# thucz/splatter360

Measured on AMD Instinct MI355X. Metric: Msplats/s fwd+bwd @1M Gaussians, 1024x512 ERP, higher is better.
Workload: dtype f32; 1 GPU; BASELINE configs[2]: 1048576 encoder-like synthetic Gaussians (seed 0, deg-4 SH, from 2 context panoramas 1024x512), 1024x512 ERP = 6 faces 256x256 + stitch, fwdbwd, L2 loss on faces (fused epilogue, scalar reduced in the backward's first launch), lean tile lists; gaussians=1048576, face=256, views_per_gpu=1, parallelism=view-sharded x1, num_rendered=2237238, visible_pairs=1096454, split_lists=auto, split_quadrants=0, wide_rectangles=0, workspace_bytes_forward=1086434304, workspace_bytes_backward=1062934272, max_instances=2862083

## Files before the change

### splatter360_amd/csrc/s360_device.h

```cpp
#pragma once
#include <hip/hip_runtime.h>
#include <stdint.h>

#include "../../include/s360.h"

#define S360_WAVE 64
#define S360_BLOCK 256

#ifndef S360_SUB_W
#define S360_SUB_W 8
#endif

static inline int s360_effective_degree(const S360Params* prm) {
    return (prm->sh_degree > 3 && (prm->flags & S360_FLAG_SH_DEG4_IGNORED)) ? 3 : prm->sh_degree;
}

#ifndef S360_PREC_F4
#define S360_PREC_F4 4
#endif

namespace s360 {

constexpr int PREC_F4 = S360_PREC_F4;
constexpr int SUB_W = S360_SUB_W, SUB_H = 64 / S360_SUB_W;
// ... 11 lines not shown
#define S360_SEG_LEN 512
#endif
#ifndef S360_SEG_HEAD
#define S360_SEG_HEAD 1024
#endif
#ifndef S360_SEG_BWD_BLOCKS
#define S360_SEG_BWD_BLOCKS 256
#endif
#ifndef S360_SEG_MIN_REST
#define S360_SEG_MIN_REST 512
#endif
constexpr uint32_t SEG_LEN = S360_SEG_LEN, SEG_HEAD = S360_SEG_HEAD, SEG_MIN_REST = S360_SEG_MIN_REST, SEG_PER_CHUNK = 4096 / SEG_LEN;
constexpr uint32_t SEG_K0 = SEG_HEAD / SEG_LEN;
static_assert(4096 % SEG_LEN == 0 && SEG_HEAD % SEG_LEN == 0 && SEG_LEN % 64 == 0 && SEG_K0 >= 1, "segments tile the sort's 4 096-key chunks; slot 0 holds the head's state");
__device__ constexpr float SEG_T_FAR = 1.0f / 16.0f;
__host__ __device__ inline size_t seg_slots(size_t cap) { return (size_t)SEG_PER_CHUNK * (cap / 2048 + 1); }
__host__ __device__ inline size_t seg_slots_of(const S360Params* prm) {
    return prm->max_segments ? (size_t)prm->max_segments : seg_slots(prm->max_instances ? prm->max_instances : 1);
}
#define S360_HDR_SPLIT 5
#define S360_HDR_SEGWORK 6
#define S360_HDR_TILES_DONE 24
#define S360_HDR_NLONG 25
#define S360_SEG_CLAIM 0x80000000u
#define S360_HDR_SEGBUFS 32

inline int device_cu_count() {
    static int cached[64] = {};
    int dev = 0;
    if (hipGetDevice(&dev) != hipSuccess || dev < 0 || dev >= 64) return 256;
    if (!cached[dev]) {
        int n = 0;
        if (hipDeviceGetAttribute(&n, hipDeviceAttributeMultiprocessorCount, dev) != hipSuccess || n <= 0) { (void)hipGetLastError(); n = 256; }
        cached[dev] = n;
    }
    return cached[dev];
}

inline int resident_blocks(const void* fn, int block_threads, int slot) {
    static int cached[64][16] = {};
    int dev = 0;
    if (hipGetDevice(&dev) != hipSuccess || dev < 0 || dev >= 64 || slot < 0 || slot >= 16) return 4 * 256;
    if (!cached[dev][slot]) {
        int per_cu = 0;
        if (hipOccupancyMaxActiveBlocksPerMultiprocessor(&per_cu, fn, block_threads, 0) != hipSuccess || per_cu <= 0) { (void)hipGetLastError(); per_cu = 4; }
        cached[dev][slot] = per_cu * device_cu_count();
// ... 573 lines not shown
```

### splatter360_amd/csrc/s360_forward.hip

```cpp
#include "s360_device.h"
#include "s360_prof.h"
#include "s360_adapter_math.h"

#include <cstdio>
#include <cstdlib>

namespace s360 {

typedef float f4v __attribute__((ext_vector_type(4)));

template <bool CH_MAJOR, bool JAC>
__global__ __launch_bounds__(S360_BLOCK) void k_sh_eval(KParams kp, const S360View* __restrict__ views,
                                                       const float* __restrict__ means, const float* __restrict__ shs,
                                                       float4* __restrict__ rgbc, float* __restrict__ sh_jac,
                                                       uint32_t* __restrict__ zero_ptr, int zero_words) {
    const int g = blockIdx.x * S360_BLOCK + threadIdx.x;
    if (g < zero_words) zero_ptr[g] = 0u;
    if (g >= kp.P) return;
    const bool fast = kp.M == 25 && kp.deg == 4;
    const float* sh = shs + (size_t)g * kp.M * 3;
    float c[75];
    if (fast) load75(sh, c);
    const S360View& vw = views[0];
    const float sc = vw.scale;
// ... 610 lines not shown
    if (lane == 63) lds[wave] = inc;
    __syncthreads();
    uint32_t base = 0, tot = 0;
#pragma unroll
    for (int w = 0; w < NW; ++w) {
        const uint32_t s = lds[w];
        if (w < wave) base += s;
        tot += s;
    }
    __syncthreads();
    total = tot;
    return base + inc - v;
}

#ifndef S360_SORT_THREADS
#define S360_SORT_THREADS 512
#endif
constexpr int SORT_THREADS = S360_SORT_THREADS;
constexpr uint32_t SORT_SHORT = 2048;
constexpr uint32_t SORT_CHUNK = 8 * SORT_THREADS;
static_assert(SORT_SHORT % SORT_THREADS == 0 && SORT_SHORT <= SORT_CHUNK, "short lists: SORT_SHORT / SORT_THREADS keys per thread");
constexpr uint32_t MAX_PASSES = 4;
__device__ __forceinline__ uint32_t ceil_log2_u32(uint32_t x) { return x <= 1 ? 0u : 32u - (uint32_t)__builtin_clz(x - 1); }
constexpr uint32_t LDSM_CHUNKS = 4;
constexpr int LDSM_E = 32;
__device__ __forceinline__ uint32_t merge_passes_of(uint32_t nch) { return nch <= 1 ? 0u : nch <= LDSM_CHUNKS ? 1u : ceil_log2_u32(nch); }

struct SegBufs {
    const uint32_t* chunk_start;
    uint32_t* seg_flag;
    uint32_t* seg_arrive;
    uint32_t* seg_arrive2;
    uint32_t n_slots;
    float4* part_c;
    float* part_t;
    float* part_e;
    uint32_t* part_l;
    uint32_t* part_n;
    float4* seg_c;
    float* seg_t;
    uint32_t* seg_cnt;
    uint2* seg_info;
    uint32_t* header;
};
static_assert(sizeof(SegBufs) <= (64 - S360_HDR_SEGBUFS) * 4, "SegBufs is parked in the workspace header");

constexpr int TS_BLOCK = 1024;
__global__ __launch_bounds__(TS_BLOCK) void k_tile_scan(const uint32_t* __restrict__ tile_count, uint32_t* __restrict__ tile_start,
                                                         uint32_t* __restrict__ tile_cursor, uint32_t* __restrict__ tile_max_contrib,
// ... 35 lines not shown
            tile_max_contrib[i1] = 0;
            chunk_start[i1] = ccarry + cex1;
        }
        carry += tot;
        ccarry += ctot;
    }
    atomicMax(&lds_max, mx);
    __syncthreads();
    if (threadIdx.x == 0) {
        chunk_start[nt] = ccarry;
        tile_start[nt] = carry;
        header[0] = carry;
        header[1] = carry > cap ? 1u : 0u;
        header[2] = lds_max;
        {
            const uint32_t nmax = min(lds_max, cap);
            const uint32_t nch = nmax > SORT_SHORT ? (nmax + SORT_CHUNK - 1) / SORT_CHUNK : 0u;
            header[3] = merge_passes_of(nch);
        }
        header[4] = 0;
        *reinterpret_cast<SegBufs*>(header + S360_HDR_SEGBUFS) = sg_in;
        header[S360_HDR_SPLIT] = 0;
        header[6] = header[7] = 0;
        if (header_mirror) __hip_atomic_store(header_mirror, (unsigned long long)carry | ((unsigned long long)(carry > cap ? 1u : 0u) << 32) |
                                                             ((unsigned long long)ccarry << 33),
                                              __ATOMIC_RELAXED, __HIP_MEMORY_SCOPE_SYSTEM);
        header[S360_HDR_NLONG] = lds_nlong;
        for (int i = 8; i < 25; ++i) header[i] = 0;
    }
}

#ifndef S360_EMIT_PPT
#define S360_EMIT_PPT 4
#endif
constexpr int EMIT_PPT = S360_EMIT_PPT;

template <bool LDS_BIN, bool COOP = false>
__global__ __launch_bounds__(S360_BLOCK) void k_emit(KParams kp, const uint32_t* __restrict__ tiles_touched,
                                                    const uint8_t* __restrict__ vis_mask, const float4* __restrict__ recA, const float4* __restrict__ recC,
                                                    const float* __restrict__ depths, const uint32_t* __restrict__ tile_start,
                                                    uint32_t* __restrict__ tile_cursor, uint64_t* __restrict__ keys,
                                                    uint2* __restrict__ slot_info, uint32_t* __restrict__ slot_pair,
                                                    uint32_t* __restrict__ slot_ticket, uint32_t* __restrict__ header,
                                                    uint32_t* __restrict__ long_pairs) {
    extern __shared__ __attribute__((aligned(16))) uint32_t lds_bin[];
    __shared__ uint32_t s_scan[S360_BLOCK / 64];
// ... 130 lines not shown
                    m = (m >> 1) | 0x80000000u;
                }
        }
        if (COOP) {
            for (unsigned long long big = __ballot(wide); big; big &= big - 1ull) {
                const int src = (int)__builtin_ctzll(big);
                const uint32_t lo = (uint32_t)__shfl((int)rlo[j], src), hi = (uint32_t)__shfl((int)rhi[j], src);
                const uint32_t ps = (uint32_t)__shfl((int)p, src), ds = (uint32_t)__shfl((int)dbits[j], src), s0 = (uint32_t)__shfl((int)slot, src);
                const uint64_t key = ((uint64_t)ds << 32) | (uint64_t)ps;
                const int minx = lo & 0xFFFFu, miny = lo >> 16, w = (int)(hi & 0xFFFFu) - minx, n = w * ((int)(hi >> 16) - miny);
                for (int i = lane; i < n; i += 64) {
                    const int y = i / w;
                    const int t = (miny + y) * kp.gx + minx + (i - y * w);
                    const uint32_t pos = LDS_BIN ? base[t] + atomicAdd(&cnt[t], 1u)
                                                 : tile_start[tb + t] + atomicAdd(&tile_cursor[tb + t], 1u);
                    if (pos < kp.cap) keys[pos] = key;
                    if (slot_pair && s0 + (uint32_t)i < kp.cap) slot_pair[s0 + (uint32_t)i] = ps | 0x80000000u;
                }
            }
        }
    }
}

template <int THREADS, int E>
__device__ __forceinline__ void block_merge_sort(const uint64_t* __restrict__ in, uint64_t* __restrict__ out,
                                                 uint32_t* __restrict__ list, uint32_t n, uint64_t* lds_m) {
#define S360_PHYS(i) ((i) + (i) / E)
    const int tid = threadIdx.x;
    uint64_t k[E];
#pragma unroll
    for (int q = 0; q < E; ++q) {
        const uint32_t i = (uint32_t)(tid * E + q);
        k[q] = i < n ? in[i] : ~0ull;
    }
#pragma unroll
    for (int r = 0; r < E; ++r) {
#pragma unroll
        for (int q = (r & 1); q + 1 < E; q += 2) {
            const uint64_t a = k[q], b = k[q + 1];
            k[q] = a < b ? a : b;
            k[q + 1] = a < b ? b : a;
        }
    }
#pragma unroll
    for (int q = 0; q < E; ++q) lds_m[S360_PHYS((uint32_t)(tid * E + q))] = k[q];
#define S360_SORT_SYNC(w)                                                      \
    do {                                                                       \
// ... 33 lines not shown
                    ka = a < width ? S360_A(a) : ~0ull;
                } else {
                    ++b;
                    kb = b < width ? S360_B(b) : ~0ull;
                }
            }
        }
        S360_SORT_SYNC(width);
        if (live) {
#pragma unroll
            for (int q = 0; q < E; ++q) lds_m[S360_PHYS(out0 + q)] = k[q];
        }
        S360_SORT_SYNC(2u * width);
#undef S360_A
#undef S360_B
    }
    __syncthreads();
#undef S360_SORT_SYNC
#pragma unroll
    for (int q = 0; q < E; ++q) {
        const uint32_t i = (uint32_t)(tid * E + q);
        if (i < n) {
            const uint64_t kq = lds_m[S360_PHYS(i)];
            out[i] = kq;
            if (list) list[i] = (uint32_t)kq;
        }
    }
#undef S360_PHYS
}



struct ChunkUnit {
    uint32_t s, n, k, passes, t;
    bool valid;
};
__device__ __forceinline__ ChunkUnit chunk_unit(const uint32_t* __restrict__ tile_start, const uint32_t* __restrict__ chunk_start,
                                                 int nt, uint32_t cap, uint32_t b) {
    ChunkUnit u;
    u.valid = b < chunk_start[nt];
    u.s = u.n = u.k = u.passes = u.t = 0;
    if (!u.valid) return u;
    const int lane = threadIdx.x & 63;
    int lo = 0, hi = nt;
    while (hi - lo > 1) {
        const int step = (hi - lo + 63) / 64;
        const int t = lo + lane * step;
        const bool p = t < hi && chunk_start[t] <= b;
        const int cnt = __popcll(__ballot(p));
        const int nhi = lo + cnt * step;
        lo = lo + (cnt - 1) * step;
        hi = nhi < hi ? nhi : hi;
    }
    u.s = min(tile_start[lo], cap);
    u.n = min(tile_start[lo + 1], cap) - u.s;
    u.k = b - chunk_start[lo];
    u.t = (uint32_t)lo;
    u.passes = merge_passes_of((u.n + SORT_CHUNK - 1) / SORT_CHUNK);
    return u;
}

__global__ __launch_bounds__(SORT_THREADS) void k_sort_stage1(const uint32_t* __restrict__ tile_start, const uint32_t* __restrict__ chunk_start,
                                                    int nt, uint64_t* __restrict__ keys, uint64_t* __restrict__ alt,
                                                    uint32_t* __restrict__ list, uint32_t cap, uint32_t max_passes, uint32_t cgrid,
                                                    const uint32_t* __restrict__ tile_count, uint32_t* __restrict__ tile_order,
                                                    const uint32_t* __restrict__ header, unsigned long long* __restrict__ wide_mirror) {
    extern __shared__ __attribute__((aligned(16))) uint64_t lds_m[];
    const uint32_t bid = blockIdx.x;
    if (bid < cgrid) {
        const uint32_t nchunks = chunk_start[nt];
        for (uint32_t b = bid; b < nchunks; b += cgrid) {
            const ChunkUnit u = chunk_unit(tile_start, chunk_start, nt, cap, b);
            if (u.valid && u.passes <= max_passes) {
                const uint32_t c0 = u.k * SORT_CHUNK, len = min(SORT_CHUNK, u.n - c0);
                uint64_t* dst = ((u.passes & 1u) ? alt : keys) + u.s + c0;
                block_merge_sort<SORT_THREADS, 8>(keys + u.s + c0, dst, u.passes == 0 ? list + u.s : nullptr, len, lds_m);
            }
            __syncthreads();
        }
        return;
    }
    if (bid < cgrid + (uint32_t)nt) {
        const uint32_t tile = bid - cgrid;
        const uint32_t s = min(tile_start[tile], cap), e = min(tile_start[tile + 1], cap);
        const uint32_t n = e - s;
        if (n == 0 || n > SORT_SHORT) return;
        block_merge_sort<SORT_THREADS, (int)(SORT_SHORT / SORT_THREADS)>(keys + s, keys + s, list + s, n, lds_m);
        return;
    }
    if (wide_mirror && threadIdx.x == 0) __hip_atomic_store(wide_mirror, (unsigned long long)header[4], __ATOMIC_RELAXED, __HIP_MEMORY_SCOPE_SYSTEM);
    if (tile_order) order_units_body<SORT_THREADS>(tile_count, tile_order, nt);
}

__device__ __forceinline__ uint64_t ld_dev(const uint64_t* p) { return __hip_atomic_load(p, __ATOMIC_RELAXED, __HIP_MEMORY_SCOPE_AGENT); }
__device__ __forceinline__ void st_dev(uint64_t* p, uint64_t v) { __hip_atomic_store(p, v, __ATOMIC_RELAXED, __HIP_MEMORY_SCOPE_AGENT); }

__device__ __forceinline__ uint32_t merge_path_global_wave(const uint64_t* __restrict__ A, uint32_t la,
                                                           const uint64_t* __restrict__ B, uint32_t lb, uint32_t d, int lane) {
    uint32_t lo = d > lb ? d - lb : 0u, hi = d < la ? d : la;
    while (lo < hi) {
        const uint32_t step = (hi - lo + 63u) / 64u;
        const uint32_t a = lo + (uint32_t)lane * step;
        const bool p = a < hi && ld_dev(A + a) <= ld_dev(B + (d - 1 - a));
        const uint32_t cnt = (uint32_t)__popcll(__ballot(p));
        if (cnt == 0) {
            hi = lo;
        } else {
            const uint32_t nhi = lo + cnt * step;
            lo = lo + (cnt - 1) * step + 1;
            hi = nhi < hi ? nhi : hi;
        }
    }
    return lo;
}

#ifndef S360_MERGE_GRID
#define S360_MERGE_GRID 256
#endif
__device__ __forceinline__ void merge_unit(const ChunkUnit& u, uint32_t pass, const uint64_t* __restrict__ keys_c, uint64_t* __restrict__ keys,
                                           uint64_t* __restrict__ alt, uint32_t* __restrict__ list, uint64_t* lds_m, uint32_t* s_part) {
    constexpr int THREADS = SORT_THREADS, E = 8;
#define S360_PHYS(i) ((i) + (i) / E)
    (void)keys_c;
    const uint32_t R = SORT_CHUNK << pass;
    const uint32_t o_tile = u.k * SORT_CHUNK, len = min(SORT_CHUNK, u.n - o_tile);
    const uint32_t pair0 = o_tile / (2 * R) * (2 * R);
    const uint32_t la = min(R, u.n - pair0), lb = min(R, u.n - pair0 - la);
    const uint64_t* src = (((u.passes - pass) & 1u) ? alt : keys) + u.s + pair0;
    uint64_t* dst = (((u.passes - pass - 1) & 1u) ? alt : keys) + u.s + o_tile;
    const uint64_t* A = src;
    const uint64_t* B = src + la;
    const uint32_t o = o_tile - pair0;
    if (threadIdx.x < 128) {
        const int w = threadIdx.x >> 6;
        const uint32_t r = merge_path_global_wave(A, la, B, lb, o + (uint32_t)w * len, threadIdx.x & 63);
        if ((threadIdx.x & 63) == 0) s_part[w] = r;
    }
    __syncthreads();
    const uint32_t a0 = s_part[0], a1 = s_part[1], b0 = o - a0, b1 = o + len - a1;
    const uint32_t na = a1 - a0, nb = b1 - b0;
    {
        uint64_t kin[E];
#pragma unroll
        for (int q = 0; q < E; ++q) {
            const uint32_t i = (uint32_t)threadIdx.x + (uint32_t)q * THREADS;
            kin[q] = i < len ? ld_dev(i < na ? A + (a0 + i) : B + (b0 + (i - na))) : 0ull;
// ... 16 lines not shown
        uint64_t ka = a < na ? lds_m[S360_PHYS(a)] : ~0ull, kb = b < nb ? lds_m[S360_PHYS(na + b)] : ~0ull;
        const bool last_pass = pass + 1 == u.passes;
        uint32_t* lst = list + u.s + o_tile;
#pragma unroll
        for (int q = 0; q < E; ++q) {
            const bool take_a = ka <= kb;
            const uint64_t kq = take_a ? ka : kb;
            if (take_a) {
                ++a;
                ka = a < na ? lds_m[S360_PHYS(a)] : ~0ull;
            } else {
                ++b;
                kb = b < nb ? lds_m[S360_PHYS(na + b)] : ~0ull;
            }
            if (out0 + q < len) {
                st_dev(dst + (out0 + q), kq);
                if (last_pass) lst[out0 + q] = (uint32_t)kq;
            }
        }
    }
#undef S360_PHYS
}

static_assert(SORT_THREADS * LDSM_E == (int)(LDSM_CHUNKS * SORT_CHUNK), "a thread merges LDSM_E outputs per pass");
constexpr size_t LDSM_LDS_BYTES = (size_t)(LDSM_CHUNKS * SORT_CHUNK + LDSM_CHUNKS * SORT_CHUNK / LDSM_E) * 8;
__device__ __forceinline__ void merge_tile_lds(uint32_t n, const uint64_t* __restrict__ src, uint64_t* __restrict__ dst, uint32_t* __restrict__ lst,
                                               uint64_t* lds_m) {
    constexpr int E = LDSM_E;
#define S360_PHYS(i) ((i) + (i) / E)
    {
        uint64_t k[E];
#pragma unroll
        for (int q = 0; q < E; ++q) {
            const uint32_t i = (uint32_t)threadIdx.x + (uint32_t)q * SORT_THREADS;
            k[q] = i < n ? src[i] : 0ull;
        }
#pragma unroll
        for (int q = 0; q < E; ++q) {
            const uint32_t i = (uint32_t)threadIdx.x + (uint32_t)q * SORT_THREADS;
            if (i < n) lds_m[S360_PHYS(i)] = k[q];
        }
    }
    __syncthreads();
    const uint32_t out0 = (uint32_t)threadIdx.x * E;
    for (uint32_t width = SORT_CHUNK; width < n; width <<= 1) {
        uint64_t k[E];
        if (out0 < n) {
            const uint32_t pa = out0 / (2 * width) * (2 * width), pb = pa + width;
            const uint32_t la = min(width, n - pa), lb = pb < n ? min(width, n - pb) : 0u;
            const uint32_t diag = out0 - pa;
            uint32_t lo = diag > lb ? diag - lb : 0u, hi = diag < la ? diag : la;
            while (lo < hi) {
                const uint32_t mid = (lo + hi) >> 1;
                if (lds_m[S360_PHYS(pa + mid)] <= lds_m[S360_PHYS(pb + (diag - 1 - mid))]) lo = mid + 1; else hi = mid;
            }
            uint32_t a = lo, b = diag - lo;
            uint64_t ka = a < la ? lds_m[S360_PHYS(pa + a)] : ~0ull, kb = b < lb ? lds_m[S360_PHYS(pb + b)] : ~0ull;
#pragma unroll
            for (int q = 0; q < E; ++q) {
                const bool take_a = ka <= kb;
                k[q] = take_a ? ka : kb;
                if (take_a) {
                    ++a;
                    ka = a < la ? lds_m[S360_PHYS(pa + a)] : ~0ull;
                } else {
                    ++b;
                    kb = b < lb ? lds_m[S360_PHYS(pb + b)] : ~0ull;
                }
            }
        }
        __syncthreads();
        if (out0 < n) {
#pragma unroll
            for (int q = 0; q < E; ++q)
                if (out0 + q < n) lds_m[S360_PHYS(out0 + q)] = k[q];
        }
        __syncthreads();
    }
    {
        uint64_t k[E];
#pragma unroll
        for (int q = 0; q < E; ++q) {
            const uint32_t i = (uint32_t)threadIdx.x + (uint32_t)q * SORT_THREADS;
            k[q] = i < n ? lds_m[S360_PHYS(i)] : 0ull;
        }
#pragma unroll
        for (int q = 0; q < E; ++q) {
            const uint32_t i = (uint32_t)threadIdx.x + (uint32_t)q * SORT_THREADS;
            if (i < n) {
                dst[i] = k[q];
                lst[i] = (uint32_t)k[q];
            }
        }
    }
#undef S360_PHYS
}

template <int THREADS>
__device__ __forceinline__ void sort_tiles_global_body(const uint32_t* __restrict__ tile_start, uint64_t* __restrict__ keys,
                                                       uint32_t* __restrict__ list, uint32_t lo, uint32_t cap, int nt) {
  for (int tile = blockIdx.x; tile < nt; tile += gridDim.x) {
    const uint32_t s = min(tile_start[tile], cap), e = min(tile_start[tile + 1], cap);
    const uint32_t n = e - s;
    if (n <= lo) continue;
    uint32_t npad = 1;
    while (npad < n) npad <<= 1;
    uint64_t* kk = keys + s;
    for (uint32_t k = 2; k <= npad; k <<= 1) {
        const uint32_t half = k >> 1;
        for (uint32_t t = threadIdx.x; t < (npad >> 1); t += THREADS) {
            const uint32_t blk = t / half, off = t - blk * half;
            const uint32_t i = blk * k + off, l = blk * k + (k - 1 - off);
            if (l < n) {
                const uint64_t a = kk[i], b = kk[l];
                if (a > b) {
                    kk[i] = b;
                    kk[l] = a;
                }
            }
        }
        __threadfence_block();
        __syncthreads();
        for (uint32_t j = k >> 2; j > 0; j >>= 1) {
            for (uint32_t t = threadIdx.x; t < (npad >> 1); t += THREADS) {
                const uint32_t i = ((t & ~(j - 1)) << 1) | (t & (j - 1)), l = i | j;
                if (l < n) {
                    const uint64_t a = kk[i], b = kk[l];
                    if (a > b) {
                        kk[i] = b;
                        kk[l] = a;
                    }
                }
            }
            __threadfence_block();
            __syncthreads();
        }
    }
    for (uint32_t i = threadIdx.x; i < n; i += THREADS) list[s + i] = (uint32_t)kk[i];
    __syncthreads();
  }
}

__global__ __launch_bounds__(SORT_THREADS) void k_merge_all(const uint32_t* __restrict__ tile_start, const uint32_t* __restrict__ chunk_start,
                                                  int nt, uint64_t* __restrict__ keys, uint64_t* __restrict__ alt,
                                                  uint32_t* __restrict__ list, uint32_t cap, uint32_t max_passes,
                                                  const uint32_t* __restrict__ header, uint32_t* __restrict__ merge_done,
                                                  uint32_t global_lo) {
    extern __shared__ __attribute__((aligned(16))) uint64_t lds_m[];
    __shared__ uint32_t s_part[2];
    __shared__ uint32_t s_ticket;
    const uint32_t npass = min(header[3], max_passes);
    const uint32_t nchunks = npass ? chunk_start[nt] : 0u;
    const uint32_t nunits = npass * nchunks;
    uint32_t* const queue = merge_done + (size_t)nt * MAX_PASSES;
    for (;;) {
        if (threadIdx.x == 0) s_ticket = nunits ? __hip_atomic_fetch_add(queue, 1u, __ATOMIC_RELAXED, __HIP_MEMORY_SCOPE_AGENT) : 0u;
        __syncthreads();
        const uint32_t tk = s_ticket;
        __syncthreads();
        if (tk >= nunits) break;
        const uint32_t pass = tk / nchunks, blk = tk - pass * nchunks;
        const ChunkUnit u = chunk_unit(tile_start, chunk_start, nt, cap, blk);
        if (!u.valid || u.passes > max_passes || pass >= u.passes) continue;
        const uint32_t nch = (u.n + SORT_CHUNK - 1) / SORT_CHUNK;
        if (nch <= LDSM_CHUNKS) {
            if (u.k == 0) merge_tile_lds(u.n, alt + u.s, keys + u.s, list + u.s, lds_m);
            continue;
        }
        if (pass > 0) {
            if (threadIdx.x == 0) {
                while (__hip_atomic_load(&merge_done[(size_t)u.t * MAX_PASSES + pass - 1], __ATOMIC_RELAXED, __HIP_MEMORY_SCOPE_AGENT) < nch)
                    __builtin_amdgcn_s_sleep(4);
            }
            __syncthreads();
        }
        merge_unit(u, pass, keys, keys, alt, list, lds_m, s_part);
        asm volatile("s_waitcnt vmcnt(0)" ::: "memory");
        __builtin_amdgcn_fence(__ATOMIC_RELEASE, "workgroup");
        __syncthreads();
        if (threadIdx.x == 0 && pass + 1 < u.passes)
            __hip_atomic_fetch_add(&merge_done[(size_t)u.t * MAX_PASSES + pass], 1u, __ATOMIC_RELAXED, __HIP_MEMORY_SCOPE_AGENT);
    }
    if (header[2] > global_lo) sort_tiles_global_body<SORT_THREADS>(tile_start, keys, list, global_lo, cap, nt);
}

#ifndef S360_SPARSE_PIXELS
#define S360_SPARSE_PIXELS 6
#endif
constexpr int SPARSE_PIXELS = S360_SPARSE_PIXELS;

struct MseEp {
    const float* target;
    float* d_images;
    float* partials;
    float grad_scale;
    float* loss_out;
};

__global__ __launch_bounds__(MSE_BLOCK) void k_mse_finish(const float* __restrict__ partials, int n_per_view, int V, float loss_scale,
                                                         float inv_elems, float* __restrict__ out) {
    mse_finish_body(partials, n_per_view, V, loss_scale, inv_elems, out);
}


__device__ __forceinline__ void st_dev32(uint32_t* p, uint32_t v) { __hip_atomic_store(p, v, __ATOMIC_RELAXED, __HIP_MEMORY_SCOPE_AGENT); }
__device__ __forceinline__ uint32_t ld_dev32(const uint32_t* p) { return __hip_atomic_load(p, __ATOMIC_RELAXED, __HIP_MEMORY_SCOPE_AGENT); }
// ... 183 lines not shown
    }
}

template <bool WITH_DEPTH, bool COH>
__device__ __forceinline__ void seg_item(const KParams& kp, const S360View* __restrict__ views, const uint32_t* __restrict__ tile_start,
                                         const uint32_t* __restrict__ list, const float4* __restrict__ recA, float* __restrict__ images,
                                         float* __restrict__ final_T, uint32_t* __restrict__ n_contrib, uint32_t* __restrict__ tile_max_contrib,
                                         uint32_t* __restrict__ strip_last, const float* __restrict__ depths, float* __restrict__ depth_maps,
                                         int depth_mode, const MseEp& ep, float4* __restrict__ surv, uint32_t* __restrict__ surv_count,
                                         const SegBufs& sg, int nt, uint32_t* __restrict__ dbg, const WaveLds& L, int lane, uint2 item, uint32_t wi,
                                         uint32_t nwork);

#ifndef S360_SPLIT_WAVES
#define S360_SPLIT_WAVES 4
#endif
#ifndef S360_P1_GRID
#define S360_P1_GRID 1024
#endif
#ifndef S360_P1_FIRST
#define S360_P1_FIRST 0
#endif
#ifndef S360_P2_GRID
#define S360_P2_GRID 1024
#endif
#ifndef S360_SEGS_SPINS
#define S360_SEGS_SPINS 600
#endif
template <bool WITH_DEPTH, bool SPLIT>
__global__ __launch_bounds__(S360_BLOCK) __attribute__((amdgpu_waves_per_eu(SPLIT ? S360_SPLIT_WAVES : 6, SPLIT ? S360_SPLIT_WAVES : 6))) void k_render(KParams kp, const S360View* __restrict__ views,
                                                      const uint32_t* __restrict__ tile_start, const uint32_t* __restrict__ list,
                                                      const float4* __restrict__ recA, const float4* __restrict__ recB,
                                                      const float4* __restrict__ recC, float* __restrict__ images,
                                                      float* __restrict__ final_T, uint32_t* __restrict__ n_contrib,
                                                      uint32_t* __restrict__ tile_max_contrib, uint32_t* __restrict__ strip_last,
                                                      uint32_t* __restrict__ dbg, const float* __restrict__ depths,
                                                      float* __restrict__ depth_maps, int depth_mode, MseEp ep,
                                                      const uint32_t* __restrict__ tile_order, float4* __restrict__ surv,
                                                      uint32_t* __restrict__ surv_count, uint32_t* __restrict__ hdr_loss,
                                                      const SegBufs* __restrict__ sgp, const uint32_t* __restrict__ chunk_start,
                                                      unsigned long long* __restrict__ cand_mirror, int nt, const uint32_t* __restrict__ list_all,
                                                      const float* __restrict__ depths_all) {
#ifdef S360_DBG_TIMING
    const long long t_begin = wall_clock64();
#endif
    __shared__ __attribute__((aligned(16))) float s_x[S360_BLOCK / 64][68], s_y[S360_BLOCK / 64][68], s_a[S360_BLOCK / 64][68],
        s_b[S360_BLOCK / 64][68], s_c[S360_BLOCK / 64][68], s_o[S360_BLOCK / 64][68];
    __shared__ __attribute__((aligned(16))) float2 s_rg[S360_BLOCK / 64][68], s_bz[S360_BLOCK / 64][68];
    __shared__ __attribute__((aligned(16))) uint32_t s_pos[S360_BLOCK / 64][68];
    if (hdr_loss && blockIdx.x == 0 && threadIdx.x == 0) {
// ... 651 lines not shown
    const size_t np = (size_t)prm->V * (size_t)(prm->P > 0 ? prm->P : 1);
    const size_t gx = (prm->W + 15) / 16, gy = (prm->H + 15) / 16;
    const size_t nt = (size_t)prm->V * gx * gy;
    const size_t cap = prm->max_instances ? prm->max_instances : 1;
    const size_t npix = (size_t)prm->V * prm->H * prm->W;
    const bool fwd_only = (prm->flags & S360_FLAG_FORWARD_ONLY) != 0;
    size_t o = 0;
    auto take = [&](size_t bytes) {
        size_t r = o;
        o = align_up(o + bytes);
        return r;
    };
    out->header = take(64 * 4);
    out->tiles_touched = take(np * 4);
    out->vis_mask = take((size_t)(prm->P > 0 ? prm->P : 1));
    out->slot_base = take(np * 8);
    out->rec_a = take(np * 48);
    out->rec_b = out->rec_a + 16;
    out->rec_c = out->rec_a + 32;
    out->clamped = take(np);
    out->depths = take(np * 4);
    out->tile_count = take(nt * 4);
    out->slot_ticket = take((size_t)prm->V * 256);
    out->merge_done = take((nt * MAX_PASSES + 1) * 4);
    out->seg_flag = take(nt * 4 * 4);
    out->seg_arrive = take(nt * 4 * 4);
    out->seg_arrive2 = take((nt * 4 + 1) * 4);
    out->tile_start = take((nt + 1) * 4);
    out->tile_cursor = take(nt * 4);
    out->chunk_start = take((nt + 1) * 4);
    out->tile_order = take(nt * 4);
    out->keys = take(cap * 8);
    out->keys_alt = take(cap * 8);
    out->list = take(cap * 4);
    out->final_T = take(npix * 4);
    out->n_contrib = take(npix * 4);
    out->tile_max_contrib = take(nt * 4);
    out->strip_last = take(nt * 4 * 4);
    out->slot_pair = take(cap * 4);
    out->long_pairs = take(fwd_only ? 16 : (cap / 32 + 1) * 4);
    out->rgbc = take((size_t)(prm->P > 0 ? prm->P : 1) * 16);
    out->sh_jac = take((size_t)(prm->P > 0 ? prm->P : 1) * 36);
    out->surv = take(fwd_only ? 16 : cap * 4 * 48);
    out->surv_count = take(nt * 4 * 4);
    {
        const bool split = (prm->flags & S360_FLAG_SPLIT_LISTS) != 0;
        const size_t ns = split ? seg_slots_of(prm) : 1, nl = ns * 4 * 64;
// ... 159 lines not shown
    if (kp.P > 0) {
        const dim3 egrid((kp.P + S360_BLOCK * EMIT_PPT - 1) / (S360_BLOCK * EMIT_PPT), kp.V);
        uint32_t* slot_pair = (kp.flags & S360_FLAG_FORWARD_ONLY) ? nullptr : (uint32_t*)(ws + L.slot_pair);
        {
        ProfScope ps(PS_EMIT, st);
        if ((size_t)kp.T * 8 <= 64 * 1024 && (kp.flags & S360_FLAG_COOP_WALK))
            hipLaunchKernelGGL((k_emit<true, true>), egrid, dim3(S360_BLOCK), (size_t)kp.T * 8, st, kp, tiles_touched, vis_mask, recA, recC,
                               depths, tile_start, tile_cursor, keys, slot_info, slot_pair, slot_ticket, header, (uint32_t*)(ws + L.long_pairs));
        else if ((size_t)kp.T * 8 <= 64 * 1024)
            hipLaunchKernelGGL(k_emit<true>, egrid, dim3(S360_BLOCK), (size_t)kp.T * 8, st, kp, tiles_touched, vis_mask, recA, recC,
                               depths, tile_start, tile_cursor, keys, slot_info, slot_pair, slot_ticket, header, (uint32_t*)(ws + L.long_pairs));
        else
            hipLaunchKernelGGL(k_emit<false>, egrid, dim3(S360_BLOCK), 0, st, kp, tiles_touched, vis_mask, recA, recC, depths, tile_start,
                               tile_cursor, keys, slot_info, slot_pair, slot_ticket, header, (uint32_t*)(ws + L.long_pairs));
        }
        S360_CHECK_LAUNCH();
        ProfScope ps(PS_SORT, st);
        {
            const size_t cap_keys = kp.cap < (uint32_t)kp.P ? kp.cap : (size_t)kp.P;
            uint32_t passes = 0;
            while (passes < MAX_PASSES && ((size_t)SORT_CHUNK << passes) < cap_keys) ++passes;
            const uint32_t global_lo = SORT_CHUNK << passes;
            const unsigned cgrid = (unsigned)min((size_t)1024, (size_t)kp.cap / SORT_CHUNK + (size_t)kp.cap / SORT_SHORT + 2);
            const size_t lds512 = (size_t)(SORT_CHUNK + SORT_CHUNK / 8) * 8;
            hipLaunchKernelGGL(k_sort_stage1, dim3(cgrid + nt + 1), dim3(SORT_THREADS), lds512, st, tile_start, chunk_start, nt, keys, keys_alt, list,
                               kp.cap, passes, cgrid, tile_count, tile_order, header,
                               prm->header_mirror ? (unsigned long long*)prm->header_mirror + 2 : (unsigned long long*)nullptr);
            if (passes > 0) {
                const unsigned mgrid = cgrid < (unsigned)S360_MERGE_GRID ? cgrid : (unsigned)S360_MERGE_GRID;
                {
                    static bool attr_done[64] = {};
                    int dev = 0;
                    if (hipGetDevice(&dev) == hipSuccess && dev >= 0 && dev < 64 && !attr_done[dev]) {
                        (void)hipFuncSetAttribute((const void*)k_merge_all, hipFuncAttributeMaxDynamicSharedMemorySize, (int)LDSM_LDS_BYTES);
                        (void)hipGetLastError();
                        attr_done[dev] = true;
                    }
                }
                hipLaunchKernelGGL(k_merge_all, dim3(mgrid), dim3(SORT_THREADS), LDSM_LDS_BYTES, st, tile_start, chunk_start, nt, keys, keys_alt, list,
                                   kp.cap, passes, header, (uint32_t*)(ws + L.merge_done), (size_t)global_lo < cap_keys ? global_lo : 0xFFFFFFFFu);
            }
        }
        S360_CHECK_LAUNCH();
    }
    {
        ProfScope ps(PS_RENDER, st);
        const dim3 rgrid(nt), rblock(S360_BLOCK);
        const bool training = !(kp.flags & S360_FLAG_FORWARD_ONLY);
        float4* surv = training ? (float4*)(ws + L.surv) : nullptr;
        uint32_t* surv_count = training ? (uint32_t*)(ws + L.surv_count) : nullptr;
#ifdef S360_DBG_TIMING
        uint32_t* dbg = (uint32_t*)keys_alt;
#else
        uint32_t* dbg = header + 8;
#endif
        const bool defer = training && kp.P > 0 && ep.target && ep.loss_out && (kp.flags & S360_FLAG_DEFER_LOSS);
        uint32_t* hdr_loss = defer ? header + S360_HDR_LOSS : nullptr;
        const bool split = kp.P > 0 && (kp.flags & S360_FLAG_SPLIT_LISTS);
        SegBufs sg{split ? chunk_start : (const uint32_t*)nullptr, (uint32_t*)(ws + L.seg_flag), (uint32_t*)(ws + L.seg_arrive),
                   (uint32_t*)(ws + L.seg_arrive2), (uint32_t)seg_slots_of(prm),
                   (float4*)(ws + L.part_c), (float*)(ws + L.part_t), (float*)(ws + L.part_e), (uint32_t*)(ws + L.part_l), (uint32_t*)(ws + L.part_n),
                   (float4*)(ws + L.seg_c), (float*)(ws + L.seg_t), (uint32_t*)(ws + L.seg_cnt), (uint2*)(ws + L.seg_info), header};
        unsigned long long* cand = prm->header_mirror ? (unsigned long long*)prm->header_mirror + 1 : nullptr;
        const SegBufs* sgp = split ? (const SegBufs*)(header + S360_HDR_SEGBUFS) : (const SegBufs*)nullptr;
// ... 75 lines not shown
```

### splatter360_amd/rasterizer.py

```python
from __future__ import annotations

import ctypes as C
import os
from typing import NamedTuple, Optional

import torch
from torch import Tensor, nn

from . import _lib

VIEW_FLOATS = 44

SH_DEG4_IGNORED = bool(int(os.environ.get("S360_SH_DEG4_IGNORED", "0")))


class GaussianRasterizationSettings(NamedTuple):
    image_height: int
    image_width: int
    tanfovx: float
    tanfovy: float
    bg: Tensor
    scale_modifier: float
    viewmatrix: Tensor
    projmatrix: Tensor
# ... 237 lines not shown

    def count_contributions(self):
        out = torch.zeros(2, dtype=torch.int64, device=self.workspace.device)
        with torch.cuda.device(self.workspace.device):
            stream = C.c_void_p(torch.cuda.current_stream(self.workspace.device).cuda_stream)
            _lib.check(_lib.lib().s360_count_contributions(C.byref(self.prm), _ptr(self.workspace), self.layout.total_bytes, _ptr(out), stream),
                       "s360_count_contributions")
        a, b = out.cpu().tolist()
        return int(a), int(b)

    def count_backward_slots(self) -> dict:
        out = torch.zeros(32, dtype=torch.int64, device=self.workspace.device)
        with torch.cuda.device(self.workspace.device):
            stream = C.c_void_p(torch.cuda.current_stream(self.workspace.device).cuda_stream)
            _lib.check(_lib.lib().s360_count_backward_slots(C.byref(self.prm), _ptr(self.workspace), self.layout.total_bytes, _ptr(out), stream),
                       "s360_count_backward_slots")
        c = [int(x) for x in out.cpu().tolist()]
        return dict(executed=c[0], padding=c[1], stopped=c[2], miss=c[3], contributing=c[4], skipped_runs=c[5], units=c[6], groups=c[7],
                    by_unit_hit_decile=c[8:18], runs_by_active_records=dict(zip(("0", "1-4", "5-8", "9-16", "17-24", "25-32", "33-48", "49-64"), c[18:26])),
                    records=c[29], reach_upper_half=c[26], reach_lower_half=c[27], reach_both_halves=c[28], half_wave_iterations=c[30])

    def split_errors(self) -> int:
        return int(self.header()[7].item())

    def mopup_items(self) -> int:
        n = int(self.header()[6].item())
        if n == 0:
            return 0
        second = self._arr(self.layout.seg_info, 2 * n, torch.int32).view(n, 2)[:, 1].to(torch.int64)
        return int(((second & 0x80000000) == 0).sum().item())

    def num_rendered(self) -> int:
        return self._read_header()[0]

    def overflowed(self) -> bool:
        return self._read_header()[1]


def _ptr(t: Optional[Tensor]):
    return None if t is None else C.c_void_p(t.data_ptr())


def _f32c(t: Tensor, name: str) -> Tensor:
    if not t.is_cuda:
        raise RuntimeError(f"{name} must live on the GPU (hip device); the rasteriser has no CPU path")
    return t.detach().float().contiguous()
# ... 502 lines not shown
```

Baseline: 1359 Msplats/s.

## Fuse chunk sort and merge passes into one persistent kernel with per-tile readiness counters

Folds the separate merge kernel into the stage-1 sort launch. Dedicated merge blocks now spin on per-tile counters of sorted chunks, so merging of a long tile can begin as soon as its chunks are sorted rather than after a kernel boundary. The LDS-resident small-merge path (merge_tile_lds) is removed, and every multi-chunk tile now goes through the global merge-path passes. Spin timeouts record an error in the header, which adds a risk of aborted merges or of deadlock if merge blocks are resident while chunk blocks are not yet scheduled.

Result: faster. 1380 Msplats/s, median of 6 (+1.5%).

```diff
diff --git a/splatter360_amd/csrc/s360_device.h b/splatter360_amd/csrc/s360_device.h
--- a/splatter360_amd/csrc/s360_device.h
+++ b/splatter360_amd/csrc/s360_device.h
@@ -57,6 +57,8 @@
 #define S360_HDR_SEGWORK 6
 #define S360_HDR_TILES_DONE 24
 #define S360_HDR_NLONG 25
+#define S360_HDR_SORT_ERR_TILE 26
+#define S360_HDR_SORT_ERR_PASS 27
 #define S360_SEG_CLAIM 0x80000000u
 #define S360_HDR_SEGBUFS 32
 
diff --git a/splatter360_amd/csrc/s360_forward.hip b/splatter360_amd/csrc/s360_forward.hip
--- a/splatter360_amd/csrc/s360_forward.hip
+++ b/splatter360_amd/csrc/s360_forward.hip
@@ -656,9 +656,10 @@
 static_assert(SORT_SHORT % SORT_THREADS == 0 && SORT_SHORT <= SORT_CHUNK, "short lists: SORT_SHORT / SORT_THREADS keys per thread");
 constexpr uint32_t MAX_PASSES = 4;
 __device__ __forceinline__ uint32_t ceil_log2_u32(uint32_t x) { return x <= 1 ? 0u : 32u - (uint32_t)__builtin_clz(x - 1); }
-constexpr uint32_t LDSM_CHUNKS = 4;
-constexpr int LDSM_E = 32;
-__device__ __forceinline__ uint32_t merge_passes_of(uint32_t nch) { return nch <= 1 ? 0u : nch <= LDSM_CHUNKS ? 1u : ceil_log2_u32(nch); }
+__device__ __forceinline__ uint32_t merge_passes_of(uint32_t nch) { return ceil_log2_u32(nch); }
+#ifndef S360_SEGS_SPINS
+#define S360_SEGS_SPINS 600
+#endif
 
 struct SegBufs {
     const uint32_t* chunk_start;
@@ -740,6 +741,7 @@
         *reinterpret_cast<SegBufs*>(header + S360_HDR_SEGBUFS) = sg_in;
         header[S360_HDR_SPLIT] = 0;
         header[6] = header[7] = 0;
+        header[S360_HDR_SORT_ERR_TILE] = header[S360_HDR_SORT_ERR_PASS] = 0;
         if (header_mirror) __hip_atomic_store(header_mirror, (unsigned long long)carry | ((unsigned long long)(carry > cap ? 1u : 0u) << 32) |
                                                              ((unsigned long long)ccarry << 33),
                                               __ATOMIC_RELAXED, __HIP_MEMORY_SCOPE_SYSTEM);
@@ -916,7 +918,10 @@
     }
 }
 
-template <int THREADS, int E>
+__device__ __forceinline__ uint64_t ld_dev(const uint64_t* p) { return __hip_atomic_load(p, __ATOMIC_RELAXED, __HIP_MEMORY_SCOPE_AGENT); }
+__device__ __forceinline__ void st_dev(uint64_t* p, uint64_t v) { __hip_atomic_store(p, v, __ATOMIC_RELAXED, __HIP_MEMORY_SCOPE_AGENT); }
+
+template <int THREADS, int E, bool DEV = false>
 __device__ __forceinline__ void block_merge_sort(const uint64_t* __restrict__ in, uint64_t* __restrict__ out,
                                                  uint32_t* __restrict__ list, uint32_t n, uint64_t* lds_m) {
 #define S360_PHYS(i) ((i) + (i) / E)
@@ -996,13 +1001,12 @@
         const uint32_t i = (uint32_t)(tid * E + q);
         if (i < n) {
             const uint64_t kq = lds_m[S360_PHYS(i)];
-            out[i] = kq;
+            if (DEV) st_dev(out + i, kq); else out[i] = kq;
             if (list) list[i] = (uint32_t)kq;
         }
     }
 #undef S360_PHYS
 }
-
 
 
 struct ChunkUnit {
@@ -1034,41 +1038,6 @@
     return u;
 }
 
-__global__ __launch_bounds__(SORT_THREADS) void k_sort_stage1(const uint32_t* __restrict__ tile_start, const uint32_t* __restrict__ chunk_start,
-                                                    int nt, uint64_t* __restrict__ keys, uint64_t* __restrict__ alt,
-                                                    uint32_t* __restrict__ list, uint32_t cap, uint32_t max_passes, uint32_t cgrid,
-                                                    const uint32_t* __restrict__ tile_count, uint32_t* __restrict__ tile_order,
-                                                    const uint32_t* __restrict__ header, unsigned long long* __restrict__ wide_mirror) {
-    extern __shared__ __attribute__((aligned(16))) uint64_t lds_m[];
-    const uint32_t bid = blockIdx.x;
-    if (bid < cgrid) {
-        const uint32_t nchunks = chunk_start[nt];
-        for (uint32_t b = bid; b < nchunks; b += cgrid) {
-            const ChunkUnit u = chunk_unit(tile_start, chunk_start, nt, cap, b);
-            if (u.valid && u.passes <= max_passes) {
-                const uint32_t c0 = u.k * SORT_CHUNK, len = min(SORT_CHUNK, u.n - c0);
-                uint64_t* dst = ((u.passes & 1u) ? alt : keys) + u.s + c0;
-                block_merge_sort<SORT_THREADS, 8>(keys + u.s + c0, dst, u.passes == 0 ? list + u.s : nullptr, len, lds_m);
-            }
-            __syncthreads();
-        }
-        return;
-    }
-    if (bid < cgrid + (uint32_t)nt) {
-        const uint32_t tile = bid - cgrid;
-        const uint32_t s = min(tile_start[tile], cap), e = min(tile_start[tile + 1], cap);
-        const uint32_t n = e - s;
-        if (n == 0 || n > SORT_SHORT) return;
-        block_merge_sort<SORT_THREADS, (int)(SORT_SHORT / SORT_THREADS)>(keys + s, keys + s, list + s, n, lds_m);
-        return;
-    }
-    if (wide_mirror && threadIdx.x == 0) __hip_atomic_store(wide_mirror, (unsigned long long)header[4], __ATOMIC_RELAXED, __HIP_MEMORY_SCOPE_SYSTEM);
-    if (tile_order) order_units_body<SORT_THREADS>(tile_count, tile_order, nt);
-}
-
-__device__ __forceinline__ uint64_t ld_dev(const uint64_t* p) { return __hip_atomic_load(p, __ATOMIC_RELAXED, __HIP_MEMORY_SCOPE_AGENT); }
-__device__ __forceinline__ void st_dev(uint64_t* p, uint64_t v) { __hip_atomic_store(p, v, __ATOMIC_RELAXED, __HIP_MEMORY_SCOPE_AGENT); }
-
 __device__ __forceinline__ uint32_t merge_path_global_wave(const uint64_t* __restrict__ A, uint32_t la,
                                                            const uint64_t* __restrict__ B, uint32_t lb, uint32_t d, int lane) {
     uint32_t lo = d > lb ? d - lb : 0u, hi = d < la ? d : la;
@@ -1088,14 +1057,10 @@
     return lo;
 }
 
-#ifndef S360_MERGE_GRID
-#define S360_MERGE_GRID 256
-#endif
-__device__ __forceinline__ void merge_unit(const ChunkUnit& u, uint32_t pass, const uint64_t* __restrict__ keys_c, uint64_t* __restrict__ keys,
+__device__ __forceinline__ void merge_unit(const ChunkUnit& u, uint32_t pass, uint64_t* __restrict__ keys,
                                            uint64_t* __restrict__ alt, uint32_t* __restrict__ list, uint64_t* lds_m, uint32_t* s_part) {
     constexpr int THREADS = SORT_THREADS, E = 8;
 #define S360_PHYS(i) ((i) + (i) / E)
-    (void)keys_c;
     const uint32_t R = SORT_CHUNK << pass;
     const uint32_t o_tile = u.k * SORT_CHUNK, len = min(SORT_CHUNK, u.n - o_tile);
     const uint32_t pair0 = o_tile / (2 * R) * (2 * R);
@@ -1158,84 +1123,11 @@
 #undef S360_PHYS
 }
 
-static_assert(SORT_THREADS * LDSM_E == (int)(LDSM_CHUNKS * SORT_CHUNK), "a thread merges LDSM_E outputs per pass");
-constexpr size_t LDSM_LDS_BYTES = (size_t)(LDSM_CHUNKS * SORT_CHUNK + LDSM_CHUNKS * SORT_CHUNK / LDSM_E) * 8;
-__device__ __forceinline__ void merge_tile_lds(uint32_t n, const uint64_t* __restrict__ src, uint64_t* __restrict__ dst, uint32_t* __restrict__ lst,
-                                               uint64_t* lds_m) {
-    constexpr int E = LDSM_E;
-#define S360_PHYS(i) ((i) + (i) / E)
-    {
-        uint64_t k[E];
-#pragma unroll
-        for (int q = 0; q < E; ++q) {
-            const uint32_t i = (uint32_t)threadIdx.x + (uint32_t)q * SORT_THREADS;
-            k[q] = i < n ? src[i] : 0ull;
-        }
-#pragma unroll
-        for (int q = 0; q < E; ++q) {
-            const uint32_t i = (uint32_t)threadIdx.x + (uint32_t)q * SORT_THREADS;
-            if (i < n) lds_m[S360_PHYS(i)] = k[q];
-        }
-    }
-    __syncthreads();
-    const uint32_t out0 = (uint32_t)threadIdx.x * E;
-    for (uint32_t width = SORT_CHUNK; width < n; width <<= 1) {
-        uint64_t k[E];
-        if (out0 < n) {
-            const uint32_t pa = out0 / (2 * width) * (2 * width), pb = pa + width;
-            const uint32_t la = min(width, n - pa), lb = pb < n ? min(width, n - pb) : 0u;
-            const uint32_t diag = out0 - pa;
-            uint32_t lo = diag > lb ? diag - lb : 0u, hi = diag < la ? diag : la;
-            while (lo < hi) {
-                const uint32_t mid = (lo + hi) >> 1;
-                if (lds_m[S360_PHYS(pa + mid)] <= lds_m[S360_PHYS(pb + (diag - 1 - mid))]) lo = mid + 1; else hi = mid;
-            }
-            uint32_t a = lo, b = diag - lo;
-            uint64_t ka = a < la ? lds_m[S360_PHYS(pa + a)] : ~0ull, kb = b < lb ? lds_m[S360_PHYS(pb + b)] : ~0ull;
-#pragma unroll
-            for (int q = 0; q < E; ++q) {
-                const bool take_a = ka <= kb;
-                k[q] = take_a ? ka : kb;
-                if (take_a) {
-                    ++a;
-                    ka = a < la ? lds_m[S360_PHYS(pa + a)] : ~0ull;
-                } else {
-                    ++b;
-                    kb = b < lb ? lds_m[S360_PHYS(pb + b)] : ~0ull;
-                }
-            }
-        }
-        __syncthreads();
-        if (out0 < n) {
-#pragma unroll
-            for (int q = 0; q < E; ++q)
-                if (out0 + q < n) lds_m[S360_PHYS(out0 + q)] = k[q];
-        }
-        __syncthreads();
-    }
-    {
-        uint64_t k[E];
-#pragma unroll
-        for (int q = 0; q < E; ++q) {
-            const uint32_t i = (uint32_t)threadIdx.x + (uint32_t)q * SORT_THREADS;
-            k[q] = i < n ? lds_m[S360_PHYS(i)] : 0ull;
-        }
-#pragma unroll
-        for (int q = 0; q < E; ++q) {
-            const uint32_t i = (uint32_t)threadIdx.x + (uint32_t)q * SORT_THREADS;
-            if (i < n) {
-                dst[i] = k[q];
-                lst[i] = (uint32_t)k[q];
-            }
-        }
-    }
-#undef S360_PHYS
-}
-
 template <int THREADS>
 __device__ __forceinline__ void sort_tiles_global_body(const uint32_t* __restrict__ tile_start, uint64_t* __restrict__ keys,
-                                                       uint32_t* __restrict__ list, uint32_t lo, uint32_t cap, int nt) {
-  for (int tile = blockIdx.x; tile < nt; tile += gridDim.x) {
+                                                       uint32_t* __restrict__ list, uint32_t lo, uint32_t cap, int nt,
+                                                       uint32_t first, uint32_t stride) {
+  for (int tile = (int)first; tile < nt; tile += (int)stride) {
     const uint32_t s = min(tile_start[tile], cap), e = min(tile_start[tile + 1], cap);
     const uint32_t n = e - s;
     if (n <= lo) continue;
@@ -1277,47 +1169,94 @@
   }
 }
 
-__global__ __launch_bounds__(SORT_THREADS) void k_merge_all(const uint32_t* __restrict__ tile_start, const uint32_t* __restrict__ chunk_start,
-                                                  int nt, uint64_t* __restrict__ keys, uint64_t* __restrict__ alt,
-                                                  uint32_t* __restrict__ list, uint32_t cap, uint32_t max_passes,
-                                                  const uint32_t* __restrict__ header, uint32_t* __restrict__ merge_done,
-                                                  uint32_t global_lo) {
+#ifndef S360_MERGE_BLOCKS
+#define S360_MERGE_BLOCKS 256
+#endif
+__device__ __forceinline__ bool wait_count(const uint32_t* counter, uint32_t need) {
+    uint32_t spins = 0;
+    while (__hip_atomic_load(counter, __ATOMIC_RELAXED, __HIP_MEMORY_SCOPE_AGENT) < need) {
+        if (++spins > (uint32_t)S360_SEGS_SPINS) return false;
+        __builtin_amdgcn_s_sleep(32);
+    }
+    return true;
+}
+__device__ __forceinline__ void drain_stores_and_sync() {
+    asm volatile("s_waitcnt vmcnt(0)" ::: "memory");
+    __builtin_amdgcn_fence(__ATOMIC_RELEASE, "workgroup");
+    __syncthreads();
+}
+__global__ __launch_bounds__(SORT_THREADS) void k_sort_stage1(const uint32_t* __restrict__ tile_start, const uint32_t* __restrict__ chunk_start,
+                                                    int nt, uint64_t* __restrict__ keys, uint64_t* __restrict__ alt,
+                                                    uint32_t* __restrict__ list, uint32_t cap, uint32_t max_passes, uint32_t cgrid,
+                                                    const uint32_t* __restrict__ tile_count, uint32_t* __restrict__ tile_order,
+                                                    uint32_t* __restrict__ header, unsigned long long* __restrict__ wide_mirror,
+                                                    uint32_t* __restrict__ merge_done, uint32_t mgrid, uint32_t global_lo) {
     extern __shared__ __attribute__((aligned(16))) uint64_t lds_m[];
-    __shared__ uint32_t s_part[2];
-    __shared__ uint32_t s_ticket;
-    const uint32_t npass = min(header[3], max_passes);
-    const uint32_t nchunks = npass ? chunk_start[nt] : 0u;
-    const uint32_t nunits = npass * nchunks;
     uint32_t* const queue = merge_done + (size_t)nt * MAX_PASSES;
-    for (;;) {
-        if (threadIdx.x == 0) s_ticket = nunits ? __hip_atomic_fetch_add(queue, 1u, __ATOMIC_RELAXED, __HIP_MEMORY_SCOPE_AGENT) : 0u;
-        __syncthreads();
-        const uint32_t tk = s_ticket;
-        __syncthreads();
-        if (tk >= nunits) break;
-        const uint32_t pass = tk / nchunks, blk = tk - pass * nchunks;
-        const ChunkUnit u = chunk_unit(tile_start, chunk_start, nt, cap, blk);
-        if (!u.valid || u.passes > max_passes || pass >= u.passes) continue;
-        const uint32_t nch = (u.n + SORT_CHUNK - 1) / SORT_CHUNK;
-        if (nch <= LDSM_CHUNKS) {
-            if (u.k == 0) merge_tile_lds(u.n, alt + u.s, keys + u.s, list + u.s, lds_m);
-            continue;
-        }
-        if (pass > 0) {
+    uint32_t* const chunks_sorted = queue + 1;
+    const uint32_t bid = blockIdx.x;
+    if (bid < cgrid) {
+        const uint32_t nchunks = chunk_start[nt];
+        for (uint32_t b = bid; b < nchunks; b += cgrid) {
+            const ChunkUnit u = chunk_unit(tile_start, chunk_start, nt, cap, b);
+            if (u.valid && u.passes <= max_passes) {
+                const uint32_t c0 = u.k * SORT_CHUNK, len = min(SORT_CHUNK, u.n - c0);
+                uint64_t* dst = ((u.passes & 1u) ? alt : keys) + u.s + c0;
+                if (u.passes == 0) {
+                    block_merge_sort<SORT_THREADS, 8>(keys + u.s + c0, dst, list + u.s, len, lds_m);
+                } else {
+                    block_merge_sort<SORT_THREADS, 8, true>(keys + u.s + c0, dst, nullptr, len, lds_m);
+                    drain_stores_and_sync();
+                    if (threadIdx.x == 0) __hip_atomic_fetch_add(&chunks_sorted[u.t], 1u, __ATOMIC_RELAXED, __HIP_MEMORY_SCOPE_AGENT);
+                }
+            }
+            __syncthreads();
+        }
+        return;
+    }
+    if (bid < cgrid + mgrid) {
+        __shared__ uint32_t s_part[2];
+        __shared__ uint32_t s_ticket;
+        const uint32_t npass = min(header[3], max_passes);
+        const uint32_t nchunks = npass ? chunk_start[nt] : 0u;
+        const uint32_t nunits = npass * nchunks;
+        while (bid - cgrid < nunits) {
+            if (threadIdx.x == 0) s_ticket = __hip_atomic_fetch_add(queue, 1u, __ATOMIC_RELAXED, __HIP_MEMORY_SCOPE_AGENT);
+            __syncthreads();
+            const uint32_t tk = s_ticket;
+            __syncthreads();
+            if (tk >= nunits) break;
+            const uint32_t pass = tk / nchunks, blk = tk - pass * nchunks;
+            const ChunkUnit u = chunk_unit(tile_start, chunk_start, nt, cap, blk);
+            if (!u.valid || u.passes > max_passes || pass >= u.passes) continue;
+            const uint32_t nch = (u.n + SORT_CHUNK - 1) / SORT_CHUNK;
             if (threadIdx.x == 0) {
-                while (__hip_atomic_load(&merge_done[(size_t)u.t * MAX_PASSES + pass - 1], __ATOMIC_RELAXED, __HIP_MEMORY_SCOPE_AGENT) < nch)
-                    __builtin_amdgcn_s_sleep(4);
+                const bool ok = wait_count(pass ? &merge_done[(size_t)u.t * MAX_PASSES + pass - 1] : &chunks_sorted[u.t], nch);
+                if (!ok && atomicAdd(&header[7], 0x1000000u) < 0x1000000u) { header[S360_HDR_SORT_ERR_TILE] = u.t; header[S360_HDR_SORT_ERR_PASS] = pass; }
+                s_ticket = ok ? 1u : 0u;
             }
             __syncthreads();
-        }
-        merge_unit(u, pass, keys, keys, alt, list, lds_m, s_part);
-        asm volatile("s_waitcnt vmcnt(0)" ::: "memory");
-        __builtin_amdgcn_fence(__ATOMIC_RELEASE, "workgroup");
-        __syncthreads();
-        if (threadIdx.x == 0 && pass + 1 < u.passes)
-            __hip_atomic_fetch_add(&merge_done[(size_t)u.t * MAX_PASSES + pass], 1u, __ATOMIC_RELAXED, __HIP_MEMORY_SCOPE_AGENT);
-    }
-    if (header[2] > global_lo) sort_tiles_global_body<SORT_THREADS>(tile_start, keys, list, global_lo, cap, nt);
+            const bool ok = s_ticket != 0u;
+            __syncthreads();
+            if (!ok) return;
+            merge_unit(u, pass, keys, alt, list, lds_m, s_part);
+            drain_stores_and_sync();
+            if (threadIdx.x == 0 && pass + 1 < u.passes)
+                __hip_atomic_fetch_add(&merge_done[(size_t)u.t * MAX_PASSES + pass], 1u, __ATOMIC_RELAXED, __HIP_MEMORY_SCOPE_AGENT);
+        }
+        if (header[2] > global_lo) sort_tiles_global_body<SORT_THREADS>(tile_start, keys, list, global_lo, cap, nt, bid - cgrid, mgrid);
+        return;
+    }
+    if (bid < cgrid + mgrid + (uint32_t)nt) {
+        const uint32_t tile = bid - cgrid - mgrid;
+        const uint32_t s = min(tile_start[tile], cap), e = min(tile_start[tile + 1], cap);
+        const uint32_t n = e - s;
+        if (n == 0 || n > SORT_SHORT) return;
+        block_merge_sort<SORT_THREADS, (int)(SORT_SHORT / SORT_THREADS)>(keys + s, keys + s, list + s, n, lds_m);
+        return;
+    }
+    if (wide_mirror && threadIdx.x == 0) __hip_atomic_store(wide_mirror, (unsigned long long)header[4], __ATOMIC_RELAXED, __HIP_MEMORY_SCOPE_SYSTEM);
+    if (tile_order) order_units_body<SORT_THREADS>(tile_count, tile_order, nt);
 }
 
 #ifndef S360_SPARSE_PIXELS
@@ -1547,9 +1486,6 @@
 #endif
 #ifndef S360_P2_GRID
 #define S360_P2_GRID 1024
-#endif
-#ifndef S360_SEGS_SPINS
-#define S360_SEGS_SPINS 600
 #endif
 template <bool WITH_DEPTH, bool SPLIT>
 __global__ __launch_bounds__(S360_BLOCK) __attribute__((amdgpu_waves_per_eu(SPLIT ? S360_SPLIT_WAVES : 6, SPLIT ? S360_SPLIT_WAVES : 6))) void k_render(KParams kp, const S360View* __restrict__ views,
@@ -2247,7 +2183,7 @@
     out->depths = take(np * 4);
     out->tile_count = take(nt * 4);
     out->slot_ticket = take((size_t)prm->V * 256);
-    out->merge_done = take((nt * MAX_PASSES + 1) * 4);
+    out->merge_done = take((nt * MAX_PASSES + 1 + nt) * 4);
     out->seg_flag = take(nt * 4 * 4);
     out->seg_arrive = take(nt * 4 * 4);
     out->seg_arrive2 = take((nt * 4 + 1) * 4);
@@ -2453,24 +2389,12 @@
             while (passes < MAX_PASSES && ((size_t)SORT_CHUNK << passes) < cap_keys) ++passes;
             const uint32_t global_lo = SORT_CHUNK << passes;
             const unsigned cgrid = (unsigned)min((size_t)1024, (size_t)kp.cap / SORT_CHUNK + (size_t)kp.cap / SORT_SHORT + 2);
+            const unsigned mgrid = passes == 0 ? 0u : cgrid < (unsigned)S360_MERGE_BLOCKS ? cgrid : (unsigned)S360_MERGE_BLOCKS;
             const size_t lds512 = (size_t)(SORT_CHUNK + SORT_CHUNK / 8) * 8;
-            hipLaunchKernelGGL(k_sort_stage1, dim3(cgrid + nt + 1), dim3(SORT_THREADS), lds512, st, tile_start, chunk_start, nt, keys, keys_alt, list,
+            hipLaunchKernelGGL(k_sort_stage1, dim3(cgrid + mgrid + nt + 1), dim3(SORT_THREADS), lds512, st, tile_start, chunk_start, nt, keys, keys_alt, list,
                                kp.cap, passes, cgrid, tile_count, tile_order, header,
-                               prm->header_mirror ? (unsigned long long*)prm->header_mirror + 2 : (unsigned long long*)nullptr);
-            if (passes > 0) {
-                const unsigned mgrid = cgrid < (unsigned)S360_MERGE_GRID ? cgrid : (unsigned)S360_MERGE_GRID;
-                {
-                    static bool attr_done[64] = {};
-                    int dev = 0;
-                    if (hipGetDevice(&dev) == hipSuccess && dev >= 0 && dev < 64 && !attr_done[dev]) {
-                        (void)hipFuncSetAttribute((const void*)k_merge_all, hipFuncAttributeMaxDynamicSharedMemorySize, (int)LDSM_LDS_BYTES);
-                        (void)hipGetLastError();
-                        attr_done[dev] = true;
-                    }
-                }
-                hipLaunchKernelGGL(k_merge_all, dim3(mgrid), dim3(SORT_THREADS), LDSM_LDS_BYTES, st, tile_start, chunk_start, nt, keys, keys_alt, list,
-                                   kp.cap, passes, header, (uint32_t*)(ws + L.merge_done), (size_t)global_lo < cap_keys ? global_lo : 0xFFFFFFFFu);
-            }
+                               prm->header_mirror ? (unsigned long long*)prm->header_mirror + 2 : (unsigned long long*)nullptr,
+                               (uint32_t*)(ws + L.merge_done), mgrid, (size_t)global_lo < cap_keys ? global_lo : 0xFFFFFFFFu);
         }
         S360_CHECK_LAUNCH();
     }
diff --git a/splatter360_amd/rasterizer.py b/splatter360_amd/rasterizer.py
--- a/splatter360_amd/rasterizer.py
+++ b/splatter360_amd/rasterizer.py
@@ -283,6 +283,9 @@
 
     def split_errors(self) -> int:
         return int(self.header()[7].item())
+
+    def sort_errors(self) -> int:
+        return int(self.header()[7].item()) >> 24
 
     def mopup_items(self) -> int:
         n = int(self.header()[6].item())
```
